# althonos/pyhmmer

Measured on AMD Instinct MI355X. Metric: GCUPS (DP cells/s) + seqs/s for hmmsearch, Pfam-A vs proteome, 1/2/4/8 GPUs, higher is better.
Workload: dtype u8/i16 filters (MSV, Viterbi), f32 Forward/Backward

## Files before the change

pyhmmer_amd/csrc/p7x_internal.hpp:

```cpp
#pragma once
#include "../../include/p7x.h"
#include <cstdint>
#include <string>
#include <vector>

namespace p7x {

constexpr int MAXK  = 20;
constexpr int MAXKP = 29;
constexpr double kLog2  = 0.69314718055994529;
constexpr double kLog2R = 1.44269504088896341;

enum { XE = 0, XN = 1, XJ = 2, XC = 3 };
enum { MOVE = 0, LOOP = 1 };
enum { tBM = 0, tMM, tIM, tDM, tMD, tMI, tII, tDD, NTRANS };
enum { gMM = 0, gIM, gDM, gBM, gMD, gDD, gMI, gII };

struct Alphabet {
  int type, K, Kp;
  const char *sym;
  unsigned char degen[MAXKP][MAXK];
  static const Alphabet &get(int type);
};

struct Profile {
  int M = 0, K = 0, Kp = 0, abc_type = 0, L = 0, max_length = -1, mode = 0;
  float nj = 1.0f;
  double relent_mh = 0.0;
  std::string name, acc, desc, consensus, rf, mm, cs;
  bool has_acc = false, has_desc = false;
  float evparam[6], cutoff[6], compo[MAXK], bgf[MAXK];
  std::vector<float> tsc;
  std::vector<float> msc;
  float xsc[4][2];
  std::vector<uint8_t> rb;
  uint8_t tbm_b, tec_b, tjb_b, base_b, bias_b;
  float scale_b;
  std::vector<int16_t> rw;
  std::vector<int16_t> tw;
  int16_t xw[4][2];
  float scale_w; int16_t base_w, ddbound_w; float ncj_roundoff;
  std::vector<float> rf_;
  std::vector<float> tf;
  float xf[4][2];

  int Q16() const { int q = (M - 1) / 16 + 1; return q < 2 ? 2 : q; }
  int Q8()  const { int q = (M - 1) / 8  + 1; return q < 2 ? 2 : q; }
  int Q4()  const { int q = (M - 1) / 4  + 1; return q < 2 ? 2 : q; }
};

float  sse_expf(float x);
uint8_t unbiased_byteify(float scale_b, float sc);
int16_t wordify(float scale_w, float sc);
double gumbel_surv(double x, double mu, double lambda);
double exp_surv(double x, double mu, double lambda);
double exp_logsurv(double x, double mu, double lambda);
float  null1_score(int L);
double match_relent_sum(const float *mat, const float *bg_f, int M, int K);
void   flogsum_init();
float  flogsum(float a, float b);

void set_error(const std::string &msg);

enum { OPT_SMALL_BLOCK = 0, OPT_VIT_WAVE, OPT_MSV_EXACT, OPT_MSV_LONG_GROUPS, OPT_MSV_BLOCKS_PER_CU, OPT_ENV_WORKSPACE_GB, OPT_DEVICE_CLUSTERED,
       OPT_TRACE_FINISH, OPT_TRACE_LONGTARGET, OPT_TRACE_ENVELOPE, OPT_HOST_PROFILE, OPT_SSV_KERNEL, OPT_MSV_F16, OPT_ENS_LDS_KB, OPT_ENS_FAIL, OPT_MSV_TIERS, OPT_STAGE_MERGE, OPT_EARLY_PACK, OPT_HOST_ORDER, OPT_VIT_LONG_CUT, OPT_FWD_GROUPED, OPT_REGION_GUARD_PPM, OPT_MSV_K8, OPT_MSV_LANE_BLOCKS, OPT_HOST_ALIGN, OPT_ALIGN_WORKSPACE_GB, OPT_CASCADE_STREAMS, OPT_CASCADE_SPLIT, OPT_SSV_PARTS, OPT_ALIGN_LOGSPACE, OPT_COUNT };
int debug_opt(int which);

}
struct p7x_oprofile;
namespace p7x {
void attach_dev_cache(p7x_oprofile *om);

}

struct p7x_oprofile { p7x::Profile p; void *dev_cache = nullptr; };
```

pyhmmer_amd/csrc/p7x_profile.cpp:

```cpp
#include "p7x_internal.hpp"
#include <atomic>
#include <algorithm>
#include <cmath>
#include <cstdio>
#include <cstring>
#include <memory>
#include <mutex>

namespace p7x {
std::atomic<int> g_debug_opt[OPT_COUNT];
static const bool g_debug_opt_ready = [] { for (auto &o : g_debug_opt) o.store(-1); return true; }();
int debug_opt(int which) { return (which >= 0 && which < OPT_COUNT) ? g_debug_opt[which].load(std::memory_order_relaxed) : -1; }


static thread_local std::string g_err;
void set_error(const std::string &msg) { g_err = msg; }

static Alphabet make_alphabet(int type)
{
  Alphabet a{};
  a.type = type;
  std::memset(a.degen, 0, sizeof(a.degen));
  if (type == P7X_AMINO) {
    a.K = 20; a.Kp = 29; a.sym = "ACDEFGHIKLMNPQRSTVWY-BJZOUX*~";
    struct { int x; const char *set; } d[] = { {21, "ND"}, {22, "IL"}, {23, "QE"}, {24, "K"}, {25, "C"} };
    for (auto &e : d) for (const char *c = e.set; *c; ++c) a.degen[e.x][std::strchr(a.sym, *c) - a.sym] = 1;
    for (int y = 0; y < 20; ++y) a.degen[26][y] = 1;
  } else {
    a.K = 4; a.Kp = 18; a.sym = (type == P7X_RNA) ? "ACGU-RYMKSWHBVDN*~" : "ACGT-RYMKSWHBVDN*~";
    const char *ref = "ACGT";
    struct { int x; const char *set; } d[] = { {5, "AG"}, {6, "CT"}, {7, "AC"}, {8, "GT"}, {9, "CG"}, {10, "AT"},
                                               {11, "ACT"}, {12, "CGT"}, {13, "ACG"}, {14, "AGT"}, {15, "ACGT"} };
    for (auto &e : d) for (const char *c = e.set; *c; ++c) a.degen[e.x][std::strchr(ref, *c) - ref] = 1;
  }
  for (int x = 0; x < a.K; ++x) a.degen[x][x] = 1;
  return a;
}

const Alphabet &Alphabet::get(int type)
{
  static const Alphabet amino = make_alphabet(P7X_AMINO), dna = make_alphabet(P7X_DNA), rna = make_alphabet(P7X_RNA);
  return type == P7X_AMINO ? amino : (type == P7X_RNA ? rna : dna);
}

float sse_expf(float x)
{
  static const float P0 = 1.9875691500E-4f, P1 = 1.3981999507E-3f, P2 = 8.3334519073E-3f,
                     P3 = 4.1665795894E-2f, P4 = 1.6666665459E-1f, P5 = 5.0000001201E-1f;
  static const float C1 = 0.693359375f, C2 = -2.12194440e-4f;
  const bool over = x > 88.72283905206835f, under = x <= -103.27892990343185f;
  if (std::isnan(x)) return x;
  if (over)  return INFINITY;
  if (under) return 0.0f;
  volatile float fx = x * (float) kLog2R;
  fx = fx + 0.5f;
  volatile float fl = (float) (int) fx;
  if (fl > fx) fl = fl - 1.0f;
  const int k = (int) fl;
  volatile float r = x;
  volatile float t1 = fl * C1, t2 = fl * C2;
  r = r - t1;
  r = r - t2;
  volatile float z = r * r;
  volatile float y = P0;
  y = y * r; y = y + P1;
  y = y * r; y = y + P2;
  y = y * r; y = y + P3;
  y = y * r; y = y + P4;
  y = y * r; y = y + P5;
  y = y * z;
  y = y + r;
  y = y + 1.0f;
  union { int32_t i; float f; } two_k;
  two_k.i = (int32_t) ((uint32_t) (k + 127) << 23);
  y = y * two_k.f;
  return y;
}

uint8_t unbiased_byteify(float scale_b, float sc)
{
  sc = -1.0f * roundf(scale_b * sc);
  return (sc > 255.) ? 255 : (uint8_t) (int) sc;
}
static uint8_t biased_byteify(float scale_b, int bias_b, float sc)
{
  sc = -1.0f * roundf(scale_b * sc);
  return (sc > 255 - bias_b) ? 255 : (uint8_t) ((int) sc + bias_b);
}
int16_t wordify(float scale_w, float sc)
{
  sc = roundf(scale_w * sc);
  if (sc >= 32767.0) return 32767;
  if (sc <= -32768.0) return -32768;
  return (int16_t) sc;
}

double gumbel_surv(double x, double mu, double lambda)
{
  const double y = lambda * (x - mu), ey = -std::exp(-y);
  return (std::fabs(ey) < 5e-9) ? -ey : 1 - std::exp(ey);
}
double exp_surv(double x, double mu, double lambda)    { return x < mu ? 1.0 : std::exp(-lambda * (x - mu)); }
double exp_logsurv(double x, double mu, double lambda) { return x < mu ? 0.0 : -lambda * (x - mu); }

float null1_score(int L)
{
  const float p1 = (float) L / (float) (L + 1);
  return (float) L * std::log((double) p1) + std::log(1. - p1);
}

static float g_flogsum[16000];
static std::once_flag g_flogsum_once;
void flogsum_init()
{
  std::call_once(g_flogsum_once, [] {
    for (int i = 0; i < 16000; ++i) g_flogsum[i] = std::log(1. + std::exp((double) -i / 1000.0));
  });
}
float flogsum(float a, float b)
{
  const float mx = a > b ? a : b, mn = a > b ? b : a;
  return (mn == -INFINITY || (mx - mn) >= 15.7f) ? mx : mx + g_flogsum[(int) ((mx - mn) * 1000.0f)];
}

static void configure_generic(Profile &p, const p7x_hmm_view &h)
{
  const Alphabet &abc = Alphabet::get(p.abc_type);
  const int M = p.M, K = p.K, Kp = p.Kp;
  const float *t = h.t;
  p.tsc.assign((size_t) (M + 1) * 8, -INFINITY);
  p.msc.assign((size_t) Kp * (M + 1), -INFINITY);
  std::vector<float> occ(M + 1);
  occ[0] = 0.f;
  occ[1] = t[0 * 7 + 1] + t[0 * 7 + 0];
  for (int k = 2; k <= M; ++k)
    occ[k] = occ[k - 1] * (t[(k - 1) * 7 + 0] + t[(k - 1) * 7 + 1]) + (1.0 - occ[k - 1]) * t[(k - 1) * 7 + 5];
  float Z = 0.f;
  for (int k = 1; k <= M; ++k) Z += occ[k] * (float) (M - k + 1);
  for (int k = 1; k <= M; ++k) p.tsc[(size_t) (k - 1) * 8 + gBM] = std::log((double) (occ[k] / Z));
  p.xsc[XE][MOVE] = -kLog2;
  p.xsc[XE][LOOP] = -kLog2;
  p.nj = 1.0f;
  for (int k = 1; k < M; ++k) {
    float *g = &p.tsc[(size_t) k * 8];
    const float *tk = t + (size_t) k * 7;
    g[gMM] = std::log((double) tk[0]); g[gMI] = std::log((double) tk[1]); g[gMD] = std::log((double) tk[2]);
    g[gIM] = std::log((double) tk[3]); g[gII] = std::log((double) tk[4]);
    g[gDM] = std::log((double) tk[5]); g[gDD] = std::log((double) tk[6]);
  }
  for (int k = 1; k <= M; ++k) {
    float sc[MAXKP];
    for (int x = 0; x < K; ++x) sc[x] = std::log((double) h.mat[(size_t) k * K + x] / p.bgf[x]);
    sc[K] = sc[Kp - 2] = sc[Kp - 1] = -INFINITY;
    for (int x = K + 1; x <= Kp - 3; ++x) {
      float num = 0.f, den = 0.f;
      for (int y = 0; y < K; ++y) if (abc.degen[x][y]) { num += sc[y] * p.bgf[y]; den += p.bgf[y]; }
      sc[x] = num / den;
    }
    for (int x = 0; x < Kp; ++x) p.msc[(size_t) x * (M + 1) + k] = sc[x];
  }
  const float pmove = (2.0f + p.nj) / ((float) p.L + 2.0f + p.nj), ploop = 1.0f - pmove;
  p.xsc[XN][LOOP] = p.xsc[XC][LOOP] = p.xsc[XJ][LOOP] = std::log((double) ploop);
  p.xsc[XN][MOVE] = p.xsc[XC][MOVE] = p.xsc[XJ][MOVE] = std::log((double) pmove);
}

static void convert_msv(Profile &p)
{
  const int M = p.M;
  float mx = 0.0f;
  for (int x = 0; x < p.K; ++x)
    for (int k = 1; k <= M; ++k) mx = std::fmax(mx, p.msc[(size_t) x * (M + 1) + k]);
  p.scale_b = 3.0 / kLog2;
  p.base_b = 190;
  p.bias_b = unbiased_byteify(p.scale_b, -1.0 * mx);
  p.rb.assign((size_t) p.Kp * (M + 1), 255);
  for (int x = 0; x < p.Kp; ++x)
    for (int k = 1; k <= M; ++k)
      p.rb[(size_t) x * (M + 1) + k] = biased_byteify(p.scale_b, p.bias_b, p.msc[(size_t) x * (M + 1) + k]);
  p.tbm_b = unbiased_byteify(p.scale_b, logf(2.0f / ((float) M * (float) (M + 1))));
  p.tec_b = unbiased_byteify(p.scale_b, logf(0.5f));
  p.tjb_b = unbiased_byteify(p.scale_b, logf(3.0f / (float) (p.L + 3)));
}

static void convert_viterbi(Profile &p)
{
  const int M = p.M;
  p.scale_w = 500.0 / kLog2;
  p.base_w = 12000;
  p.rw.assign((size_t) p.Kp * (M + 1), -32768);
  for (int x = 0; x < p.Kp; ++x)
    for (int k = 1; k <= M; ++k) p.rw[(size_t) x * (M + 1) + k] = wordify(p.scale_w, p.msc[(size_t) x * (M + 1) + k]);
  p.tw.assign((size_t) NTRANS * (M + 1), -32768);
  auto W = [&](int t, int k) -> int16_t & { return p.tw[(size_t) t * (M + 1) + k]; };
  auto cap = [](int16_t v, int16_t maxval) { return v <= maxval ? v : maxval; };
  for (int k = 1; k <= M; ++k) {
    W(tBM, k) = cap(wordify(p.scale_w, p.tsc[(size_t) (k - 1) * 8 + gBM]), 0);
    W(tMM, k) = cap(wordify(p.scale_w, p.tsc[(size_t) (k - 1) * 8 + gMM]), 0);
    W(tIM, k) = cap(wordify(p.scale_w, p.tsc[(size_t) (k - 1) * 8 + gIM]), 0);
    W(tDM, k) = cap(wordify(p.scale_w, p.tsc[(size_t) (k - 1) * 8 + gDM]), 0);
    if (k < M) {
      W(tMD, k) = cap(wordify(p.scale_w, p.tsc[(size_t) k * 8 + gMD]), 0);
      W(tMI, k) = cap(wordify(p.scale_w, p.tsc[(size_t) k * 8 + gMI]), 0);
      W(tII, k) = cap(wordify(p.scale_w, p.tsc[(size_t) k * 8 + gII]), -1);
      W(tDD, k) = wordify(p.scale_w, p.tsc[(size_t) k * 8 + gDD]);
    }
  }
  p.xw[XE][LOOP] = wordify(p.scale_w, p.xsc[XE][LOOP]);
  p.xw[XE][MOVE] = wordify(p.scale_w, p.xsc[XE][MOVE]);
  for (int s : {XN, XC, XJ}) { p.xw[s][MOVE] = wordify(p.scale_w, p.xsc[s][MOVE]); p.xw[s][LOOP] = 0; }
  p.ncj_roundoff = 0.0f;
  int bound = -32768;
  for (int k = 2; k < M - 1; ++k) {
    int dd = (int) wordify(p.scale_w, p.tsc[(size_t) k * 8 + gDD]);
    dd += (int) wordify(p.scale_w, p.tsc[(size_t) (k + 1) * 8 + gDM]);
    dd -= (int) wordify(p.scale_w, p.tsc[(size_t) (k + 1) * 8 + gBM]);
    if (dd > bound) bound = dd;
  }
  p.ddbound_w = (int16_t) bound;
}

static void convert_forward(Profile &p)
{
  const int M = p.M;
  p.rf_.assign((size_t) p.Kp * (M + 1), 0.0f);
  for (int x = 0; x < p.Kp; ++x)
    for (int k = 1; k <= M; ++k) p.rf_[(size_t) x * (M + 1) + k] = sse_expf(p.msc[(size_t) x * (M + 1) + k]);
  p.tf.assign((size_t) NTRANS * (M + 1), 0.0f);
  auto F = [&](int t, int k) -> float & { return p.tf[(size_t) t * (M + 1) + k]; };
  for (int k = 1; k <= M; ++k) {
    F(tBM, k) = sse_expf(p.tsc[(size_t) (k - 1) * 8 + gBM]);
    F(tMM, k) = sse_expf(p.tsc[(size_t) (k - 1) * 8 + gMM]);
    F(tIM, k) = sse_expf(p.tsc[(size_t) (k - 1) * 8 + gIM]);
    F(tDM, k) = sse_expf(p.tsc[(size_t) (k - 1) * 8 + gDM]);
    if (k < M) {
      F(tMD, k) = sse_expf(p.tsc[(size_t) k * 8 + gMD]);
      F(tMI, k) = sse_expf(p.tsc[(size_t) k * 8 + gMI]);
      F(tII, k) = sse_expf(p.tsc[(size_t) k * 8 + gII]);
      F(tDD, k) = sse_expf(p.tsc[(size_t) k * 8 + gDD]);
    }
  }
  for (int s = 0; s < 4; ++s) for (int m = 0; m < 2; ++m) p.xf[s][m] = expf(p.xsc[s][m]);
}

}

using namespace p7x;

extern "C" {

int p7x_abi_version(void) { return P7X_ABI_VERSION; }

int p7x_debug_set_option(const char *name, int value)
{
  static const char *const names[p7x::OPT_COUNT] = { "small_block", "vit_wave", "msv_exact", "msv_long_groups", "msv_blocks_per_cu", "env_workspace_gb",
                                                     "device_clustered", "trace_finish", "trace_longtarget", "trace_envelope", "host_profile", "ssv_kernel", "msv_f16", "ens_lds_kb", "ens_fail", "msv_tiers", "stage_merge", "early_pack", "host_order", "vit_long_cut", "fwd_grouped", "region_guard_ppm", "msv_k8", "msv_lane_blocks", "host_align", "align_workspace_gb", "cascade_streams", "cascade_split", "ssv_parts", "align_logspace" };
  if (!name) { p7x::set_error("p7x_debug_set_option: no name"); return P7X_EINVAL; }
  for (int i = 0; i < p7x::OPT_COUNT; ++i)
    if (std::strcmp(name, names[i]) == 0) { p7x::g_debug_opt[i].store(value); return P7X_OK; }
  p7x::set_error(std::string("p7x_debug_set_option: unknown option ") + name);
  return P7X_EINVAL;
}

const char *p7x_last_error(void) { return g_err.c_str(); }

void p7x_expf_neg(const double *in, float *out, size_t n)
{
  for (size_t i = 0; i < n; ++i) out[i] = std::isinf(in[i]) ? 0.0f : expf((float) (-1.0 * in[i]));
}

int p7x_hmm_max_length(const p7x_hmm_view *h, double beta, int32_t *out)
{
  if (!h || !out || h->M < 1 || !h->t || !(beta > 0.0)) { set_error("p7x_hmm_max_length: bad arguments"); return P7X_EINVAL; }
  const int M = h->M;
  if (M == 1) { *out = 1; return P7X_OK; }
  const float *t = h->t;
  auto T = [&](int k, int x) -> double { return (double) t[(size_t) k * 7 + x]; };
  std::vector<double> Mm(2 * (size_t) (M + 1), 0.0), I(2 * (size_t) (M + 1), 0.0), D(2 * (size_t) (M + 1), 0.0);
  auto at = [&](std::vector<double> &v, int k, int c) -> double & { return v[(size_t) c * (M + 1) + k]; };
  at(Mm, 1, 0) = 1.0;
  for (int k = 2; k <= M; ++k) at(D, k, 0) = T(k - 1, 2) * at(Mm, k - 1, 0) + T(k - 1, 6) * at(D, k - 1, 0);
  const int length_bound = 200000;
  for (int L = 2; L <= length_bound; ++L) {
    const int c = (L - 1) & 1, pc = L & 1;
    at(Mm, 1, c) = 0.0; at(D, 1, c) = 0.0;
    at(I, 1, c) = T(1, 1) * at(Mm, 1, pc) + T(1, 4) * at(I, 1, pc);
    double alive = at(I, 1, c);
    for (int k = 2; k <= M; ++k) {
      const double m = T(k - 1, 0) * at(Mm, k - 1, pc) + T(k - 1, 3) * at(I, k - 1, pc) + T(k - 1, 5) * at(D, k - 1, pc);
      const double i = k < M ? T(k, 1) * at(Mm, k, pc) + T(k, 4) * at(I, k, pc) : 0.0;
      at(Mm, k, c) = m; at(I, k, c) = i;
      at(D, k, c) = T(k - 1, 2) * at(Mm, k - 1, c) + T(k - 1, 6) * at(D, k - 1, c);
      alive += m + i;
    }
    if (alive < beta) { *out = L; return P7X_OK; }
  }
  set_error("p7x_hmm_max_length: no bound below 200000 residues");
  return P7X_ERANGE;
}

int p7x_oprofile_create(const p7x_hmm_view *h, const float *bg_f, int32_t L, p7x_oprofile **out)
{
  if (!h || !bg_f || !out || h->M < 1 || !h->t || !h->mat || !h->name) { set_error("p7x_oprofile_create: bad arguments"); return P7X_EINVAL; }
  if (h->abc_type != P7X_AMINO && h->abc_type != P7X_DNA && h->abc_type != P7X_RNA) { set_error("unknown alphabet"); return P7X_EINVAL; }
  flogsum_init();
  auto *om = new p7x_oprofile();
  Profile &p = om->p;
  const Alphabet &abc = Alphabet::get(h->abc_type);
  p.M = h->M; p.K = abc.K; p.Kp = abc.Kp; p.abc_type = h->abc_type; p.L = L; p.max_length = h->max_length;
  p.mode = 1;
  p.name = h->name;
  if (h->acc)  { p.acc = h->acc;   p.has_acc = true; }
  if (h->desc) { p.desc = h->desc; p.has_desc = true; }
  if (h->consensus) p.consensus = h->consensus;
  if (h->rf) p.rf = h->rf;
  if (h->mm) p.mm = h->mm;
  if (h->cs) p.cs = h->cs;
  std::memcpy(p.evparam, h->evparam, sizeof(p.evparam));
  std::memcpy(p.cutoff, h->cutoff, sizeof(p.cutoff));
  std::memset(p.compo, 0, sizeof(p.compo));
  if (h->compo) std::memcpy(p.compo, h->compo, sizeof(float) * p.K);
  std::memset(p.bgf, 0, sizeof(p.bgf));
  std::memcpy(p.bgf, bg_f, sizeof(float) * p.K);
  p.relent_mh = match_relent_sum(h->mat, bg_f, p.M, p.K);
  configure_generic(p, *h);
  convert_msv(p);
  convert_viterbi(p);
  convert_forward(p);
  attach_dev_cache(om);
  *out = om;
  return P7X_OK;
}

int p7x_oprofile_get_info(const p7x_oprofile *om, p7x_oprofile_info *o)
{
  if (!om || !o) return P7X_EINVAL;
  const Profile &p = om->p;
  std::memset(o, 0, sizeof(*o));
  o->M = p.M; o->K = p.K; o->Kp = p.Kp; o->abc_type = p.abc_type; o->L = p.L; o->max_length = p.max_length; o->mode = p.mode;
  o->Q16 = p.Q16(); o->Q8 = p.Q8(); o->Q4 = p.Q4();
  o->tbm_b = p.tbm_b; o->tec_b = p.tec_b; o->tjb_b = p.tjb_b; o->base_b = p.base_b; o->bias_b = p.bias_b; o->scale_b = p.scale_b;
  std::memcpy(o->xw, p.xw, sizeof(p.xw));
  o->scale_w = p.scale_w; o->base_w = p.base_w; o->ddbound_w = p.ddbound_w; o->ncj_roundoff = p.ncj_roundoff;
  std::memcpy(o->xf, p.xf, sizeof(p.xf));
  std::memcpy(o->evparam, p.evparam, sizeof(p.evparam));
  std::memcpy(o->cutoff, p.cutoff, sizeof(p.cutoff));
  std::memcpy(o->compo, p.compo, sizeof(p.compo));
  o->nj = p.nj;
  return P7X_OK;
}

int64_t p7x_oprofile_striped(const p7x_oprofile *om, int which, void *out, size_t out_bytes)
{
  if (!om || !out) return -1;
  const Profile &p = om->p;
  const int M = p.M, Kp = p.Kp;
  auto node = [](int q, int z, int Q) { return q + 1 + z * Q; };
  switch (which) {
  case 0: {
    const int Q = p.Q16(); const size_t need = (size_t) Kp * Q * 16;
    if (out_bytes < need) return -1;
    auto *o = (uint8_t *) out;
    for (int x = 0; x < Kp; ++x) for (int q = 0; q < Q; ++q) for (int z = 0; z < 16; ++z) {
      const int k = node(q, z, Q);
      o[((size_t) x * Q + q) * 16 + z] = k <= M ? p.rb[(size_t) x * (M + 1) + k] : 255;
    }
    return (int64_t) need;
  }
  case 1: {
    const int Q = p.Q16(), QS = Q + 17; const size_t need = (size_t) Kp * QS * 16;
    if (out_bytes < need) return -1;
    auto *o = (int8_t *) out;
    const uint8_t top = (uint8_t) (p.bias_b + 127);
    for (int x = 0; x < Kp; ++x) for (int q = 0; q < QS; ++q) for (int z = 0; z < 16; ++z) {
      const int k = node(q % Q, z, Q);
      const uint8_t r = k <= M ? p.rb[(size_t) x * (M + 1) + k] : 255;
      const uint8_t d = top > r ? (uint8_t) (top - r) : 0;
      o[((size_t) x * QS + q) * 16 + z] = (int8_t) (d ^ 127);
    }
    return (int64_t) need;
  }
  case 2: {
    const int Q = p.Q8(); const size_t need = (size_t) Kp * Q * 8 * 2;
    if (out_bytes < need) return -1;
    auto *o = (int16_t *) out;
    for (int x = 0; x < Kp; ++x) for (int q = 0; q < Q; ++q) for (int z = 0; z < 8; ++z) {
      const int k = node(q, z, Q);
      o[((size_t) x * Q + q) * 8 + z] = k <= M ? p.rw[(size_t) x * (M + 1) + k] : -32768;
    }
    return (int64_t) need;
  }
  case 3: {
    const int Q = p.Q8(); const size_t need = (size_t) 8 * Q * 8 * 2;
    if (out_bytes < need) return -1;
    auto *o = (int16_t *) out;
    for (int q = 0; q < Q; ++q) for (int z = 0; z < 8; ++z) {
      const int k = node(q, z, Q);
      for (int t = tBM; t <= tII; ++t) {
        int16_t v = k <= M ? p.tw[(size_t) t * (M + 1) + k] : -32768;
        if (k > M) v = (t == tII) ? -32768 : -32768;
        o[((size_t) q * 7 + t) * 8 + z] = v;
      }
      o[((size_t) 7 * Q + q) * 8 + z] = k <= M ? p.tw[(size_t) tDD * (M + 1) + k] : -32768;
    }
    return (int64_t) need;
  }
  case 4: {
    const int Q = p.Q4(); const size_t need = (size_t) Kp * Q * 4 * 4;
    if (out_bytes < need) return -1;
    auto *o = (float *) out;
    for (int x = 0; x < Kp; ++x) for (int q = 0; q < Q; ++q) for (int z = 0; z < 4; ++z) {
      const int k = node(q, z, Q);
      o[((size_t) x * Q + q) * 4 + z] = k <= M ? p.rf_[(size_t) x * (M + 1) + k] : 0.0f;
    }
    return (int64_t) need;
  }
  case 5: {
    const int Q = p.Q4(); const size_t need = (size_t) 8 * Q * 4 * 4;
    if (out_bytes < need) return -1;
    auto *o = (float *) out;
    for (int q = 0; q < Q; ++q) for (int z = 0; z < 4; ++z) {
      const int k = node(q, z, Q);
      for (int t = tBM; t <= tII; ++t) o[((size_t) q * 7 + t) * 4 + z] = k <= M ? p.tf[(size_t) t * (M + 1) + k] : 0.0f;
      o[((size_t) 7 * Q + q) * 4 + z] = k <= M ? p.tf[(size_t) tDD * (M + 1) + k] : 0.0f;
    }
    return (int64_t) need;
  }
  default: return -1;
  }
}


}

namespace {
constexpr uint32_t kMagicF = 0xb3e6e6f3u, kMagicP = 0xb3e6f0f3u;

struct Writer {
  uint8_t *buf; size_t cap; size_t n = 0;
  void bytes(const void *p, size_t len) { if (buf && n + len <= cap) std::memcpy(buf + n, p, len); n += len; }
  template <typename T> void pod(T v) { bytes(&v, sizeof(T)); }
  void str_f(const std::string &s) { pod<int32_t>((int32_t) s.size()); bytes(s.c_str(), s.size() + 1); }
  void str_p(const std::string &s, bool have) { if (!have || s.empty()) { pod<int32_t>(0); return; } str_f(s); }
  void line(const std::string &s, int M) { std::vector<char> l((size_t) M + 2, 0); std::memcpy(l.data(), s.data(), std::min(s.size(), (size_t) M + 1)); bytes(l.data(), l.size()); }
};
struct Rd {
  const uint8_t *buf; size_t len; size_t n = 0; bool ok = true;
  void bytes(void *p, size_t k) { if (n + k > len) { ok = false; return; } std::memcpy(p, buf + n, k); n += k; }
  template <typename T> T pod() { T v{}; bytes(&v, sizeof(T)); return v; }
  std::string str(int32_t k) { std::string s; if (k < 0 || n + (size_t) k + 1 > len) { ok = false; return s; } s.assign((const char *) buf + n, (size_t) k); n += (size_t) k + 1; return s; }
  std::string line(int M) { std::string s; if (n + (size_t) M + 2 > len) { ok = false; return s; } s.assign((const char *) buf + n, strnlen((const char *) buf + n, (size_t) M + 2)); n += (size_t) M + 2; return s; }
};

void write_pressed(const Profile &p, const int64_t offs[3], Writer &f, Writer &q, const p7x_oprofile *om)
{
  const int M = p.M, Kp = p.Kp;
  std::vector<uint8_t> tmp;
  auto striped = [&](int which, size_t bytes) { tmp.resize(bytes); p7x_oprofile_striped(om, which, tmp.data(), bytes); return tmp.data(); };
  f.pod(kMagicF); f.pod<int32_t>(M); f.pod<int32_t>(p.abc_type);
  f.str_f(p.name);
  f.pod<int32_t>(p.max_length);
  f.pod(p.tbm_b); f.pod(p.tec_b); f.pod(p.tjb_b); f.pod(p.scale_b); f.pod(p.base_b); f.pod(p.bias_b);
  { const size_t n = (size_t) Kp * (p.Q16() + 17) * 16; f.bytes(striped(1, n), n); }
  { const size_t n = (size_t) Kp * p.Q16() * 16; f.bytes(striped(0, n), n); }
  f.bytes(p.evparam, sizeof(p.evparam));
  f.bytes(offs, 3 * sizeof(int64_t));
  { float compo[20]; std::memset(compo, 0, sizeof(compo)); std::memcpy(compo, p.compo, sizeof(float) * std::min(20, (int) MAXK)); f.bytes(compo, sizeof(compo)); }
  f.pod(kMagicF);
  q.pod(kMagicP); q.pod<int32_t>(M); q.pod<int32_t>(p.abc_type);
  q.str_p(p.name, true); q.str_p(p.acc, p.has_acc); q.str_p(p.desc, p.has_desc);
  q.line(p.rf, M); q.line(p.mm, M); q.line(p.cs, M); q.line(p.consensus, M);
  { const size_t n = (size_t) 8 * p.Q8() * 8 * 2; q.bytes(striped(3, n), n); }
  { const size_t n = (size_t) Kp * p.Q8() * 8 * 2; q.bytes(striped(2, n), n); }
  q.bytes(p.xw, sizeof(p.xw));
  q.pod(p.scale_w); q.pod(p.base_w); q.pod(p.ddbound_w); q.pod(p.ncj_roundoff);
  { const size_t n = (size_t) 8 * p.Q4() * 4 * 4; q.bytes(striped(5, n), n); }
  { const size_t n = (size_t) Kp * p.Q4() * 4 * 4; q.bytes(striped(4, n), n); }
  q.bytes(p.xf, sizeof(p.xf));
  q.bytes(p.cutoff, sizeof(p.cutoff));
  q.pod(p.nj); q.pod<int32_t>(p.mode); q.pod<int32_t>(p.L);
  q.pod(kMagicP);
}
}

extern "C" {

int p7x_fasta_parse(const char *text, size_t n, const uint8_t *lut, size_t *nseq, size_t *nres, size_t *strbytes,
                    uint8_t *dsq, int64_t *offsets, int32_t *lengths, char *strtab, int64_t *name_off, int64_t *desc_off,
                    size_t *bad_pos)
{
  if (!text || !lut || !nseq || !nres || !strbytes) { set_error("p7x_fasta_parse: bad arguments"); return P7X_EINVAL; }
  const bool fill = dsq != nullptr;
  if (fill && (!offsets || !lengths || !strtab || !name_off || !desc_off)) { set_error("p7x_fasta_parse: bad arguments"); return P7X_EINVAL; }
  size_t ns = 0, nr = 0, sb = 0, pos = 0, w = 0;
  if (fill) dsq[w] = 255;
  ++w;
  while (pos < n && text[pos] != '>') {
    const unsigned char c = (unsigned char) text[pos];
    if (c != ' ' && c != '\t' && c != '\r' && c != '\n') { if (bad_pos) *bad_pos = pos; set_error("FASTA text does not start with '>'"); return P7X_EFORMAT; }
    ++pos;
  }
  while (pos < n) {
    size_t h0 = pos + 1, h1 = h0;
    while (h1 < n && text[h1] != '\n') ++h1;
    size_t he = h1;
    while (he > h0 && (text[he - 1] == '\r' || text[he - 1] == ' ' || text[he - 1] == '\t')) --he;
    size_t a = h0;
    while (a < he && (text[a] == ' ' || text[a] == '\t')) ++a;
    size_t b = a;
    while (b < he && text[b] != ' ' && text[b] != '\t') ++b;
    size_t d = b;
    while (d < he && (text[d] == ' ' || text[d] == '\t')) ++d;
    if (fill) {
      name_off[ns] = (int64_t) sb; std::memcpy(strtab + sb, text + a, b - a); strtab[sb + (b - a)] = 0;
      desc_off[ns] = (int64_t) (sb + (b - a) + 1); std::memcpy(strtab + sb + (b - a) + 1, text + d, he - d); strtab[sb + (b - a) + 1 + (he - d)] = 0;
    }
    sb += (b - a) + 1 + (he - d) + 1;
    pos = h1 < n ? h1 + 1 : n;
    const size_t start = w;
    bool bol = true;
    while (pos < n) {
      const unsigned char c = (unsigned char) text[pos];
      if (bol && c == '>') break;
      if (c == '\n') { bol = true; ++pos; continue; }
      bol = false;
      const uint8_t code = lut[c];
      if (code < 254) { if (fill) dsq[w] = code; ++w; }
      else if (code == 255) { if (bad_pos) *bad_pos = pos; set_error(std::string("invalid symbol '") + (char) c + "' in sequence data"); return P7X_EFORMAT; }
      ++pos;
    }
    const size_t L = w - start;
    if (L > 0x7fffffff) { set_error("sequence too long"); return P7X_ERANGE; }
    if (fill) { offsets[ns] = (int64_t) start; lengths[ns] = (int32_t) L; dsq[w] = 255; }
    ++w;
    nr += L; ++ns;
  }
  *nseq = ns; *nres = nr; *strbytes = sb;
  return P7X_OK;
}

int p7x_oprofile_get_string(const p7x_oprofile *om, int which, char *buf, size_t n)
{
  if (!om || !buf || n == 0) return -1;
  const Profile &p = om->p;
  const std::string *s = nullptr;
  switch (which) {
    case 0: s = &p.name; break;
    case 1: if (p.has_acc) s = &p.acc; break;
    case 2: if (p.has_desc) s = &p.desc; break;
    case 3: s = &p.consensus; break;
    default: return -1;
  }
  buf[0] = 0;
  if (!s || s->empty()) return 0;
  std::snprintf(buf, n, "%s", s->c_str());
  return (int) s->size();
}

int p7x_oprofile_write_pressed(const p7x_oprofile *om, const int64_t offs[3], uint8_t *h3f, size_t cap_f, size_t *len_f,
// ... 110 lines not shown
```

pyhmmer_amd/csrc/p7x_vitpk.hip:

```cpp
#include <map>
#include "p7x_wave.hpp"
#include <mutex>

namespace p7x {

namespace {

typedef short s2v __attribute__((ext_vector_type(2)));
__device__ __forceinline__ s2v as_s2v(uint32_t u) { return __builtin_bit_cast(s2v, u); }
__device__ __forceinline__ uint32_t as_u(s2v v) { return __builtin_bit_cast(uint32_t, v); }
__device__ __forceinline__ uint32_t pk_adds(uint32_t a, uint32_t b) { return as_u(__builtin_elementwise_add_sat(as_s2v(a), as_s2v(b))); }
__device__ __forceinline__ uint32_t pk_max(uint32_t a, uint32_t b) { return as_u(__builtin_elementwise_max(as_s2v(a), as_s2v(b))); }
__device__ __forceinline__ uint32_t splat16(int v) { const uint32_t w = (uint32_t) v & 0xffffu; return w | (w << 16); }
__device__ __forceinline__ int lo_of(uint32_t w) { return (int) (short) (w & 0xffffu); }
__device__ __forceinline__ int hi_of(uint32_t w) { return (int) (short) (w >> 16); }

constexpr uint32_t kNeg2 = 0x80008000u;
constexpr int vitpk_rowq(int T, int P)
{
  const int n = ((P + 3) / 4) * T;
  return T == 8 ? ((n & 15) == 8 ? n : n + 8) : n;
}

#define P7X_DPP_U(v, ctrl) ((uint32_t) __builtin_amdgcn_update_dpp((int) kNeg2, (int) (v), (ctrl), 0xf, 0xf, false))

template <int T>
__device__ __forceinline__ int group_max(uint32_t v)
{
  v = pk_max(v, P7X_DPP_U(v, 0xB1));
  v = pk_max(v, P7X_DPP_U(v, 0x4E));
  v = pk_max(v, P7X_DPP_U(v, 0x141));
  if constexpr (T == 16) v = pk_max(v, P7X_DPP_U(v, 0x140));
  return max(lo_of(v), hi_of(v));
}

}

struct RowState { int xN, xB, xJ, xC; bool overflow; };

template <int T>
__device__ __forceinline__ uint32_t stripe_shift(uint32_t r, bool first)
{
  const uint32_t prev = P7X_DPP_U(r, 0x138);
  const uint32_t last = P7X_DPP_U(r, T == 8 ? 0x141 : 0x140);
  return first ? ((last << 16) | 0x8000u) : prev;
}

template <int T, int P>
__device__ __forceinline__ void vit_row(const VitPkArgs &a, const uint4 *tral, const uint4 *trbl, const uint4 *er, bool first,
                                        bool active, int xwm, const uint32_t (&mi)[P], const uint32_t (&ii)[P],
                                        const uint32_t (&di)[P], uint32_t (&mo_)[P], uint32_t (&io_)[P], uint32_t (&do_)[P],
                                        const uint32_t (&tdd)[P], RowState &rs)
{
  constexpr int PS = (P + 3) & ~3;
  const uint32_t xBv = splat16(rs.xB);
  uint32_t mp = stripe_shift<T>(mi[P - 1], first), ip = stripe_shift<T>(ii[P - 1], first), dp = stripe_shift<T>(di[P - 1], first);
  uint32_t xEv = kNeg2, dmaxv = kNeg2, dcv = kNeg2;
#pragma unroll
  for (int j4 = 0; j4 < PS; j4 += 4) {
    const uint4 e4 = er[(j4 / 4) * T];
    const uint32_t ev[4] = { e4.x, e4.y, e4.z, e4.w };
#pragma unroll
    for (int jj = 0; jj < 4; ++jj) {
      const int q = j4 + jj;
      if (q < P) {
        const uint4 ta = tral[q * T], tb = trbl[q * T];
        const uint32_t a0 = pk_adds(xBv, ta.x), a1 = pk_adds(mp, ta.y), a2 = pk_adds(ip, ta.z), a3 = pk_adds(dp, ta.w);
        uint32_t sv = pk_max(pk_max(a0, a1), pk_max(a2, a3));
        sv = pk_adds(sv, ev[jj]);
        xEv = pk_max(xEv, sv);
        mo_[q] = sv;
        if (q > 0) do_[q] = dcv;
        dcv = pk_adds(sv, tb.x);
        dmaxv = pk_max(dmaxv, dcv);
        io_[q] = pk_max(pk_adds(mi[q], tb.y), pk_adds(ii[q], tb.z));
        mp = mi[q]; ip = ii[q]; dp = di[q];
      }
    }
    asm volatile("" ::: "memory");
  }
  do_[0] = stripe_shift<T>(dcv, first);
  const int xE = group_max<T>(xEv);
  const int Dmax = group_max<T>(dmaxv);
  if (active) {
    if (xE >= 32767) rs.overflow = true;
    rs.xC = max(rs.xC, xE + a.xw_e);
    rs.xJ = max(rs.xJ, xE + a.xw_e);
    rs.xB = max(rs.xJ + xwm, rs.xN + xwm);
  }
  const bool trig = active && (Dmax + a.ddbound > rs.xB);
#ifdef P7X_VITPK_NO_CLOSURE
  if (false) {
#else
  if (__any(trig)) {
#endif
    int pass = 0;
    bool more;
    do {
#pragma unroll
      for (int q = 1; q < P; ++q) do_[q] = pk_max(do_[q], pk_adds(do_[q - 1], tdd[q - 1]));
      uint32_t c = stripe_shift<T>(pk_adds(do_[P - 1], tdd[P - 1]), first);
      if (!trig) c = kNeg2;
      const uint32_t d0 = pk_max(do_[0], c);
      const bool changed = d0 != do_[0];
      do_[0] = d0;
      more = __any(changed) && ++pass < 2 * T;
    } while (more);
  }
}

template <int T, int P>
__global__ void __launch_bounds__(256) vitpk_kernel(const ArgRef ref)
{
  constexpr int G = 64 / T;
  const VitPkArgs a = load_args<VitPkArgs>(ref);
  const int nlist = a.nlist_ptr ? *a.nlist_ptr : a.nlist;
  const int nskip = a.nskip_ptr ? *a.nskip_ptr : 0;
  if (nskip + (int) (blockIdx.x * 4 * G) >= nlist) return;
  constexpr int PS = (P + 3) & ~3;
  constexpr int ROWQ = vitpk_rowq(T, P);
  extern __shared__ __attribute__((aligned(16))) unsigned char smem[];
  uint4 *tra = reinterpret_cast<uint4 *>(smem);
  uint4 *trb = tra + P * T;
  uint4 *em = trb + P * T;
  {
    const uint4 *gt = reinterpret_cast<const uint4 *>(a.trans);
    for (int i = threadIdx.x; i < 2 * P * T; i += 256) tra[i] = gt[i];
    const uint4 *ge = reinterpret_cast<const uint4 *>(a.emis);
    for (int i = threadIdx.x; i < a.nrows * ROWQ; i += 256) em[i] = ge[i];
  }
  __syncthreads();
  const int lane = threadIdx.x & 63;
  const int s = lane % T, g = lane / T;
  const bool first = (s == 0);
  const int wave0 = rfl((int) (blockIdx.x * 4 + (threadIdx.x >> 6)));
  const int nwaves = (int) gridDim.x * 4;
  const uint4 *tral = tra + s, *trbl = trb + s, *eml = em + s;
  uint32_t tdd[P];
#pragma unroll
  for (int q = 0; q < P; ++q) tdd[q] = trbl[q * T].w;

  for (int it0 = nskip + wave0 * G; it0 < nlist; it0 += nwaves * G) {
    const int it = it0 + g;
    const bool have = it < nlist;
    const int slot = have ? (a.list ? a.list[it] : it) : 0;
    const int L = have ? a.slot_len[slot] : 0;
    const uint8_t *sq = a.dsq + (have ? a.slot_off[slot] : 0);
    const int xwm = (int) a.xwmove_tab[L];
    const int Lmax = wave_max_i32(L);

    uint32_t mA[P], iA[P], dA[P], mB[P], iB[P], dB[P];
#pragma unroll
    for (int j = 0; j < P; ++j) mA[j] = iA[j] = dA[j] = kNeg2;
    RowState rs;
    rs.xN = a.base_w; rs.xB = rs.xN + xwm; rs.xJ = -32768; rs.xC = -32768; rs.overflow = false;

    for (int i0 = 0; i0 < Lmax; i0 += 4 * T) {
      uint32_t word = 0;
#pragma unroll
      for (int b = 0; b < 4; ++b) {
        const int r = i0 + 4 * s + b;
        const uint32_t x = (r < L) ? (uint32_t) sq[r] : 0u;
        word |= x << (8 * b);
      }
      const int nrow = min(4 * T, Lmax - i0);
      auto residue = [&](int r) -> uint32_t {
        const uint32_t w = (uint32_t) __shfl((int) word, g * T + (r >> 2));
        return (w >> (8 * (r & 3))) & 0xffu;
      };
      int r = 0;
      for (; r + 1 < nrow; r += 2) {
        vit_row<T, P>(a, tral, trbl, eml + residue(r) * ROWQ, first, i0 + r < L, xwm, mA, iA, dA, mB, iB, dB, tdd, rs);
        vit_row<T, P>(a, tral, trbl, eml + residue(r + 1) * ROWQ, first, i0 + r + 1 < L, xwm, mB, iB, dB, mA, iA, dA, tdd, rs);
      }
      if (r < nrow) {
        vit_row<T, P>(a, tral, trbl, eml + residue(r) * ROWQ, first, i0 + r < L, xwm, mA, iA, dA, mB, iB, dB, tdd, rs);
#pragma unroll
        for (int j = 0; j < P; ++j) { mA[j] = mB[j]; iA[j] = iB[j]; dA[j] = dB[j]; }
      }
    }
    const bool overflow = rs.overflow; const int xC = rs.xC;
    if (have && s == 0) a.out_xC[it] = overflow ? 32767 : xC;
  }
}

bool vitpk_pick(int M, int *T, int *P)
{
  static const int p8[] = { 2, 4, 6, 8, 10, 12, 14, 15, 16, 17, 18, 19, 20 };
  static const int p16[] = { 11, 12, 13, 14, 15, 16, 17, 18, 19, 20 };
  for (int p : p8) if (M <= 8 * 2 * p) { *T = 8; *P = p; return true; }
  for (int p : p16) if (M <= 16 * 2 * p) { *T = 16; *P = p; return true; }
  return false;
}

void vitpk_build_tables(const Profile &p, int T, int P, std::vector<uint32_t> &trans, std::vector<uint32_t> &emis)
{
  const int rowq = vitpk_rowq(T, P), nrows = p.Kp + 1;
  auto pack = [](int lo, int hi) { return ((uint32_t) lo & 0xffffu) | (((uint32_t) hi & 0xffffu) << 16); };
  trans.assign((size_t) 2 * P * T * 4, kNeg2);
  emis.assign((size_t) nrows * rowq * 4, kNeg2);
  for (int s = 0; s < T; ++s)
    for (int j = 0; j < P; ++j) {
      const int k0 = s * P + j + 1, k1 = (s + T) * P + j + 1;
      for (int t = 0; t < NTRANS; ++t) {
        const int lo = (k0 <= p.M) ? p.tw[(size_t) t * (p.M + 1) + k0] : -32768;
        const int hi = (k1 <= p.M) ? p.tw[(size_t) t * (p.M + 1) + k1] : -32768;
        trans[((size_t) (t / 4) * P * T + (size_t) j * T + s) * 4 + (t % 4)] = pack(lo, hi);
      }
      for (int x = 0; x < p.Kp; ++x) {
        const int lo = (k0 <= p.M) ? p.rw[(size_t) x * (p.M + 1) + k0] : -32768;
        const int hi = (k1 <= p.M) ? p.rw[(size_t) x * (p.M + 1) + k1] : -32768;
        emis[((size_t) x * rowq + (size_t) (j / 4) * T + s) * 4 + (j % 4)] = pack(lo, hi);
      }
    }
}

template <int T, int P>
static int launch_pk(const ArgRun<VitPkArgs> &a, int num_cu, hipStream_t st)
{
  const size_t lds = ((size_t) 2 * P * T + (size_t) a.at(0).nrows * vitpk_rowq(T, P)) * 16;
  auto kern = vitpk_kernel<T, P>;
  static std::map<int, int> per_cu_by_device;
  static std::mutex mu;
  int per_cu = 0;
  {
    int dev = 0; P7X_HIP(hipGetDevice(&dev));
    std::lock_guard<std::mutex> lk(mu);
    int &cached = per_cu_by_device[dev];
    if (cached == 0) {
      if (lds > 64 * 1024) P7X_HIP(hipFuncSetAttribute(reinterpret_cast<const void *>(kern), hipFuncAttributeMaxDynamicSharedMemorySize, (int) lds));
      P7X_HIP(hipOccupancyMaxActiveBlocksPerMultiprocessor(&cached, kern, 256, lds));
      if (cached < 1) cached = 1;
    }
    per_cu = cached;
  }
  long want = 0;
  for (int i = 0; i < a.n; ++i) want = std::max<long>(want, ((long) a.at(i).nlist + 4 * (64 / T) - 1) / (4 * (64 / T)));
  if (want <= 0) return P7X_OK;
  hipLaunchKernelGGL(kern, dim3(lane_grid(want, (long) num_cu * per_cu, a.n), (unsigned) a.n), dim3(256), lds, st, a.ref());
  P7X_HIP(hipGetLastError());
  return P7X_OK;
}

int vitpk_launch(int T, int P, const ArgRun<VitPkArgs> &a, int num_cu, hipStream_t st)
{
  if (a.n <= 0) return P7X_OK;
#define P7X_PK(TT, PP) if (T == TT && P == PP) return launch_pk<TT, PP>(a, num_cu, st);
  P7X_PK(8, 2) P7X_PK(8, 4) P7X_PK(8, 6) P7X_PK(8, 8) P7X_PK(8, 10) P7X_PK(8, 12) P7X_PK(8, 14) P7X_PK(8, 15) P7X_PK(8, 16)
  P7X_PK(8, 17) P7X_PK(8, 18) P7X_PK(8, 19) P7X_PK(8, 20)
  P7X_PK(16, 11) P7X_PK(16, 12) P7X_PK(16, 13) P7X_PK(16, 14) P7X_PK(16, 15) P7X_PK(16, 16) P7X_PK(16, 17) P7X_PK(16, 18)
  P7X_PK(16, 19) P7X_PK(16, 20)
#undef P7X_PK
  set_error("no packed Viterbi kernel for this model length");
  return P7X_EINVAL;
}

}
```

Before: 26000.

## Extend packed i16 Viterbi kernel to 32- and 64-lane stripes for long models

Adds T=32 and T=64 variants of the packed Viterbi kernel so models longer than 640 positions can use the register-resident packed path instead of the fallback. Cross-lane reductions and stripe shifts use permlane16/32 swaps, readlane and a row-wide DPP shift. Block size now varies with the template parameters (up to 16 waves). The path is on by default and can be disabled with the vit_wide option. It adds many template instantiations and more register pressure for large P.

```diff
diff --git a/pyhmmer_amd/csrc/p7x_internal.hpp b/pyhmmer_amd/csrc/p7x_internal.hpp
--- a/pyhmmer_amd/csrc/p7x_internal.hpp
+++ b/pyhmmer_amd/csrc/p7x_internal.hpp
@@ -63,7 +63,7 @@
 void set_error(const std::string &msg);
 
 enum { OPT_SMALL_BLOCK = 0, OPT_VIT_WAVE, OPT_MSV_EXACT, OPT_MSV_LONG_GROUPS, OPT_MSV_BLOCKS_PER_CU, OPT_ENV_WORKSPACE_GB, OPT_DEVICE_CLUSTERED,
-       OPT_TRACE_FINISH, OPT_TRACE_LONGTARGET, OPT_TRACE_ENVELOPE, OPT_HOST_PROFILE, OPT_SSV_KERNEL, OPT_MSV_F16, OPT_ENS_LDS_KB, OPT_ENS_FAIL, OPT_MSV_TIERS, OPT_STAGE_MERGE, OPT_EARLY_PACK, OPT_HOST_ORDER, OPT_VIT_LONG_CUT, OPT_FWD_GROUPED, OPT_REGION_GUARD_PPM, OPT_MSV_K8, OPT_MSV_LANE_BLOCKS, OPT_HOST_ALIGN, OPT_ALIGN_WORKSPACE_GB, OPT_CASCADE_STREAMS, OPT_CASCADE_SPLIT, OPT_SSV_PARTS, OPT_ALIGN_LOGSPACE, OPT_COUNT };
+       OPT_TRACE_FINISH, OPT_TRACE_LONGTARGET, OPT_TRACE_ENVELOPE, OPT_HOST_PROFILE, OPT_SSV_KERNEL, OPT_MSV_F16, OPT_ENS_LDS_KB, OPT_ENS_FAIL, OPT_MSV_TIERS, OPT_STAGE_MERGE, OPT_EARLY_PACK, OPT_HOST_ORDER, OPT_VIT_LONG_CUT, OPT_FWD_GROUPED, OPT_REGION_GUARD_PPM, OPT_MSV_K8, OPT_MSV_LANE_BLOCKS, OPT_HOST_ALIGN, OPT_ALIGN_WORKSPACE_GB, OPT_CASCADE_STREAMS, OPT_CASCADE_SPLIT, OPT_SSV_PARTS, OPT_ALIGN_LOGSPACE, OPT_VIT_WIDE, OPT_COUNT };
 int debug_opt(int which);
 
 }
diff --git a/pyhmmer_amd/csrc/p7x_profile.cpp b/pyhmmer_amd/csrc/p7x_profile.cpp
--- a/pyhmmer_amd/csrc/p7x_profile.cpp
+++ b/pyhmmer_amd/csrc/p7x_profile.cpp
@@ -253,7 +253,7 @@
 int p7x_debug_set_option(const char *name, int value)
 {
   static const char *const names[p7x::OPT_COUNT] = { "small_block", "vit_wave", "msv_exact", "msv_long_groups", "msv_blocks_per_cu", "env_workspace_gb",
-                                                     "device_clustered", "trace_finish", "trace_longtarget", "trace_envelope", "host_profile", "ssv_kernel", "msv_f16", "ens_lds_kb", "ens_fail", "msv_tiers", "stage_merge", "early_pack", "host_order", "vit_long_cut", "fwd_grouped", "region_guard_ppm", "msv_k8", "msv_lane_blocks", "host_align", "align_workspace_gb", "cascade_streams", "cascade_split", "ssv_parts", "align_logspace" };
+                                                     "device_clustered", "trace_finish", "trace_longtarget", "trace_envelope", "host_profile", "ssv_kernel", "msv_f16", "ens_lds_kb", "ens_fail", "msv_tiers", "stage_merge", "early_pack", "host_order", "vit_long_cut", "fwd_grouped", "region_guard_ppm", "msv_k8", "msv_lane_blocks", "host_align", "align_workspace_gb", "cascade_streams", "cascade_split", "ssv_parts", "align_logspace", "vit_wide" };
   if (!name) { p7x::set_error("p7x_debug_set_option: no name"); return P7X_EINVAL; }
   for (int i = 0; i < p7x::OPT_COUNT; ++i)
     if (std::strcmp(name, names[i]) == 0) { p7x::g_debug_opt[i].store(value); return P7X_OK; }
diff --git a/pyhmmer_amd/csrc/p7x_vitpk.hip b/pyhmmer_amd/csrc/p7x_vitpk.hip
--- a/pyhmmer_amd/csrc/p7x_vitpk.hip
+++ b/pyhmmer_amd/csrc/p7x_vitpk.hip
@@ -30,7 +30,15 @@
   v = pk_max(v, P7X_DPP_U(v, 0xB1));
   v = pk_max(v, P7X_DPP_U(v, 0x4E));
   v = pk_max(v, P7X_DPP_U(v, 0x141));
-  if constexpr (T == 16) v = pk_max(v, P7X_DPP_U(v, 0x140));
+  if constexpr (T >= 16) v = pk_max(v, P7X_DPP_U(v, 0x140));
+  if constexpr (T >= 32) {
+    const auto x = __builtin_amdgcn_permlane16_swap(v, v, false, false);
+    v = pk_max(x[0], x[1]);
+  }
+  if constexpr (T == 64) {
+    const auto x = __builtin_amdgcn_permlane32_swap(v, v, false, false);
+    v = pk_max(x[0], x[1]);
+  }
   return max(lo_of(v), hi_of(v));
 }
 
@@ -39,22 +47,30 @@
 struct RowState { int xN, xB, xJ, xC; bool overflow; };
 
 template <int T>
-__device__ __forceinline__ uint32_t stripe_shift(uint32_t r, bool first)
-{
+__device__ __forceinline__ uint32_t stripe_shift(uint32_t r, bool first, bool hi)
+{
+  if constexpr (T == 64) {
+    const uint32_t w = P7X_DPP_U(r, 0x13C);
+    return first ? ((w << 16) | 0x8000u) : w;
+  }
   const uint32_t prev = P7X_DPP_U(r, 0x138);
-  const uint32_t last = P7X_DPP_U(r, T == 8 ? 0x141 : 0x140);
+  uint32_t last;
+  if constexpr (T == 32) {
+    const uint32_t l31 = (uint32_t) __builtin_amdgcn_readlane((int) r, 31), l63 = (uint32_t) __builtin_amdgcn_readlane((int) r, 63);
+    last = hi ? l63 : l31;
+  } else last = P7X_DPP_U(r, T == 8 ? 0x141 : 0x140);
   return first ? ((last << 16) | 0x8000u) : prev;
 }
 
 template <int T, int P>
-__device__ __forceinline__ void vit_row(const VitPkArgs &a, const uint4 *tral, const uint4 *trbl, const uint4 *er, bool first,
+__device__ __forceinline__ void vit_row(const VitPkArgs &a, const uint4 *tral, const uint4 *trbl, const uint4 *er, bool first, bool hi,
                                         bool active, int xwm, const uint32_t (&mi)[P], const uint32_t (&ii)[P],
                                         const uint32_t (&di)[P], uint32_t (&mo_)[P], uint32_t (&io_)[P], uint32_t (&do_)[P],
                                         const uint32_t (&tdd)[P], RowState &rs)
 {
   constexpr int PS = (P + 3) & ~3;
   const uint32_t xBv = splat16(rs.xB);
-  uint32_t mp = stripe_shift<T>(mi[P - 1], first), ip = stripe_shift<T>(ii[P - 1], first), dp = stripe_shift<T>(di[P - 1], first);
+  uint32_t mp = stripe_shift<T>(mi[P - 1], first, hi), ip = stripe_shift<T>(ii[P - 1], first, hi), dp = stripe_shift<T>(di[P - 1], first, hi);
   uint32_t xEv = kNeg2, dmaxv = kNeg2, dcv = kNeg2;
 #pragma unroll
   for (int j4 = 0; j4 < PS; j4 += 4) {
@@ -79,7 +95,7 @@
     }
     asm volatile("" ::: "memory");
   }
-  do_[0] = stripe_shift<T>(dcv, first);
+  do_[0] = stripe_shift<T>(dcv, first, hi);
   const int xE = group_max<T>(xEv);
   const int Dmax = group_max<T>(dmaxv);
   if (active) {
@@ -99,7 +115,7 @@
     do {
 #pragma unroll
       for (int q = 1; q < P; ++q) do_[q] = pk_max(do_[q], pk_adds(do_[q - 1], tdd[q - 1]));
-      uint32_t c = stripe_shift<T>(pk_adds(do_[P - 1], tdd[P - 1]), first);
+      uint32_t c = stripe_shift<T>(pk_adds(do_[P - 1], tdd[P - 1]), first, hi);
       if (!trig) c = kNeg2;
       const uint32_t d0 = pk_max(do_[0], c);
       const bool changed = d0 != do_[0];
@@ -109,14 +125,22 @@
   }
 }
 
+constexpr int vitpk_waves(int T, int P)
+{
+  if (T == 64) return P <= 12 ? 16 : 12;
+  if (T == 32) return (P >= 13 && P <= 16) ? 12 : 8;
+  return 4;
+}
+
 template <int T, int P>
-__global__ void __launch_bounds__(256) vitpk_kernel(const ArgRef ref)
+__global__ void __launch_bounds__(64 * vitpk_waves(T, P)) vitpk_kernel(const ArgRef ref)
 {
   constexpr int G = 64 / T;
+  constexpr int NW = vitpk_waves(T, P), NT = 64 * NW;
   const VitPkArgs a = load_args<VitPkArgs>(ref);
   const int nlist = a.nlist_ptr ? *a.nlist_ptr : a.nlist;
   const int nskip = a.nskip_ptr ? *a.nskip_ptr : 0;
-  if (nskip + (int) (blockIdx.x * 4 * G) >= nlist) return;
+  if (nskip + (int) (blockIdx.x * NW * G) >= nlist) return;
   constexpr int PS = (P + 3) & ~3;
   constexpr int ROWQ = vitpk_rowq(T, P);
   extern __shared__ __attribute__((aligned(16))) unsigned char smem[];
@@ -125,16 +149,16 @@
   uint4 *em = trb + P * T;
   {
     const uint4 *gt = reinterpret_cast<const uint4 *>(a.trans);
-    for (int i = threadIdx.x; i < 2 * P * T; i += 256) tra[i] = gt[i];
+    for (int i = threadIdx.x; i < 2 * P * T; i += NT) tra[i] = gt[i];
     const uint4 *ge = reinterpret_cast<const uint4 *>(a.emis);
-    for (int i = threadIdx.x; i < a.nrows * ROWQ; i += 256) em[i] = ge[i];
+    for (int i = threadIdx.x; i < a.nrows * ROWQ; i += NT) em[i] = ge[i];
   }
   __syncthreads();
   const int lane = threadIdx.x & 63;
   const int s = lane % T, g = lane / T;
-  const bool first = (s == 0);
-  const int wave0 = rfl((int) (blockIdx.x * 4 + (threadIdx.x >> 6)));
-  const int nwaves = (int) gridDim.x * 4;
+  const bool first = (s == 0), hi = (g != 0);
+  const int wave0 = rfl((int) (blockIdx.x * NW + (threadIdx.x >> 6)));
+  const int nwaves = (int) gridDim.x * NW;
   const uint4 *tral = tra + s, *trbl = trb + s, *eml = em + s;
   uint32_t tdd[P];
 #pragma unroll
@@ -170,11 +194,11 @@
       };
       int r = 0;
       for (; r + 1 < nrow; r += 2) {
-        vit_row<T, P>(a, tral, trbl, eml + residue(r) * ROWQ, first, i0 + r < L, xwm, mA, iA, dA, mB, iB, dB, tdd, rs);
-        vit_row<T, P>(a, tral, trbl, eml + residue(r + 1) * ROWQ, first, i0 + r + 1 < L, xwm, mB, iB, dB, mA, iA, dA, tdd, rs);
+        vit_row<T, P>(a, tral, trbl, eml + residue(r) * ROWQ, first, hi, i0 + r < L, xwm, mA, iA, dA, mB, iB, dB, tdd, rs);
+        vit_row<T, P>(a, tral, trbl, eml + residue(r + 1) * ROWQ, first, hi, i0 + r + 1 < L, xwm, mB, iB, dB, mA, iA, dA, tdd, rs);
       }
       if (r < nrow) {
-        vit_row<T, P>(a, tral, trbl, eml + residue(r) * ROWQ, first, i0 + r < L, xwm, mA, iA, dA, mB, iB, dB, tdd, rs);
+        vit_row<T, P>(a, tral, trbl, eml + residue(r) * ROWQ, first, hi, i0 + r < L, xwm, mA, iA, dA, mB, iB, dB, tdd, rs);
 #pragma unroll
         for (int j = 0; j < P; ++j) { mA[j] = mB[j]; iA[j] = iB[j]; dA[j] = dB[j]; }
       }
@@ -190,6 +214,11 @@
   static const int p16[] = { 11, 12, 13, 14, 15, 16, 17, 18, 19, 20 };
   for (int p : p8) if (M <= 8 * 2 * p) { *T = 8; *P = p; return true; }
   for (int p : p16) if (M <= 16 * 2 * p) { *T = 16; *P = p; return true; }
+  if (debug_opt(OPT_VIT_WIDE) == 0) return false;
+  static const int p32[] = { 11, 12, 13, 14, 15, 16, 17, 18, 19, 20 };
+  static const int p64[] = { 11, 12, 13, 14, 15, 16 };
+  for (int p : p32) if (M <= 32 * 2 * p) { *T = 32; *P = p; return true; }
+  for (int p : p64) if (M <= 64 * 2 * p) { *T = 64; *P = p; return true; }
   return false;
 }
 
@@ -220,6 +249,7 @@
 {
   const size_t lds = ((size_t) 2 * P * T + (size_t) a.at(0).nrows * vitpk_rowq(T, P)) * 16;
   auto kern = vitpk_kernel<T, P>;
+  constexpr int NW = vitpk_waves(T, P), NT = 64 * NW;
   static std::map<int, int> per_cu_by_device;
   static std::mutex mu;
   int per_cu = 0;
@@ -229,15 +259,15 @@
     int &cached = per_cu_by_device[dev];
     if (cached == 0) {
       if (lds > 64 * 1024) P7X_HIP(hipFuncSetAttribute(reinterpret_cast<const void *>(kern), hipFuncAttributeMaxDynamicSharedMemorySize, (int) lds));
-      P7X_HIP(hipOccupancyMaxActiveBlocksPerMultiprocessor(&cached, kern, 256, lds));
+      P7X_HIP(hipOccupancyMaxActiveBlocksPerMultiprocessor(&cached, kern, NT, lds));
       if (cached < 1) cached = 1;
     }
     per_cu = cached;
   }
   long want = 0;
-  for (int i = 0; i < a.n; ++i) want = std::max<long>(want, ((long) a.at(i).nlist + 4 * (64 / T) - 1) / (4 * (64 / T)));
+  for (int i = 0; i < a.n; ++i) want = std::max<long>(want, ((long) a.at(i).nlist + NW * (64 / T) - 1) / (NW * (64 / T)));
   if (want <= 0) return P7X_OK;
-  hipLaunchKernelGGL(kern, dim3(lane_grid(want, (long) num_cu * per_cu, a.n), (unsigned) a.n), dim3(256), lds, st, a.ref());
+  hipLaunchKernelGGL(kern, dim3(lane_grid(want, (long) num_cu * per_cu, a.n), (unsigned) a.n), dim3(NT), lds, st, a.ref());
   P7X_HIP(hipGetLastError());
   return P7X_OK;
 }
@@ -250,6 +280,9 @@
   P7X_PK(8, 17) P7X_PK(8, 18) P7X_PK(8, 19) P7X_PK(8, 20)
   P7X_PK(16, 11) P7X_PK(16, 12) P7X_PK(16, 13) P7X_PK(16, 14) P7X_PK(16, 15) P7X_PK(16, 16) P7X_PK(16, 17) P7X_PK(16, 18)
   P7X_PK(16, 19) P7X_PK(16, 20)
+  P7X_PK(32, 11) P7X_PK(32, 12) P7X_PK(32, 13) P7X_PK(32, 14) P7X_PK(32, 15) P7X_PK(32, 16) P7X_PK(32, 17) P7X_PK(32, 18)
+  P7X_PK(32, 19) P7X_PK(32, 20)
+  P7X_PK(64, 11) P7X_PK(64, 12) P7X_PK(64, 13) P7X_PK(64, 14) P7X_PK(64, 15) P7X_PK(64, 16)
 #undef P7X_PK
   set_error("no packed Viterbi kernel for this model length");
   return P7X_EINVAL;
```

Result: faster. 26370, median of 6 (+1.4%).
